# opencb/hpg-variant

Hardware: AMD Instinct MI355X
Metric: variants/s chi2 assoc (higher is better)
Workload: dtype u8

## Files before the change

### hpg-variant_amd/csrc/hpgv_capi.hip

```cpp
#include "hpgv_internal.h"
#include <cstdlib>

extern "C" {

const char *hpgv_version(void) { return "hpgv-mi355x 0.1 (gfx950)"; }

int hpgv_device_count(void) {
    int n = 0;
    if (hipGetDeviceCount(&n) != hipSuccess) return -1;
    return n;
}

const char *hpgv_last_error(const hpgv_ctx *ctx) { return ctx ? ctx->err.c_str() : g_create_error.c_str(); }

static void read_environment(hpgv_ctx *ctx) {
    auto num = [](const char *name, long lo, long hi, long *out) { const char *e = getenv(name); if (e && *e) { long v = atol(e); *out = v < lo ? lo : v > hi ? hi : v; } };
    num("HPGV_BATCH_COPY", 0, 1, &ctx->batch_copy);
    num("HPGV_BATCH_FUSED", 0, 1, &ctx->batch_fused);
    num("HPGV_STATS_ALL2", 0, 1, &ctx->stats_all2);
    num("HPGV_ASSOC_ROWS", 0, 1, &ctx->assoc_rows);
    num("HPGV_PINNED_NONCOHERENT", 0, 1, &ctx->pinned_noncoherent);
    num("HPGV_VMM_TRACE", 0, 1, &ctx->vmm_trace);
    num("HPGV_DECODE_TILES", 0, 1, &ctx->decode_tiles);
#ifdef HPGV_ABLATION
// ... 198 lines not shown
    } else if (!strcmp(key, "inflate_wave")) {
        if (value < 0 || value > 4) return fail(ctx, HPGV_ERR_INVALID, "inflate_wave must be 0 (lane per block), 1 (by the number of blocks), 2 (wave per block), 4 (wave per block, several symbols per round) or 3 (lane per block, symbol tables in LDS)");
        HPGV_SHIPPED_ONLY(value == 1 || value == 4, "inflate_wave other than 1 / 4 (a wave per block, several symbols per round)")
        ctx->inflate_wave = value;
    } else if (!strcmp(key, "tokenizer_tiles")) {
        if (value < 0 || value > 2) return fail(ctx, HPGV_ERR_INVALID, "tokenizer_tiles must be 2 (one sweep), 1 (two sweeps) or 0 (line by line)");
        HPGV_SHIPPED_ONLY(value == 1, "tokenizer_tiles other than 1 (two sweeps)")
        ctx->tokenizer_tiles = value;
    } else if (!strcmp(key, "fisher_width")) {
        if (value != 64 && value != 32 && value != 16 && value != 8) return fail(ctx, HPGV_ERR_INVALID, "fisher_width must be 64, 32, 16 or 8");
        HPGV_SHIPPED_ONLY(value == 16, "fisher_width other than 16")
        ctx->fisher_width = value;
    } else if (!strcmp(key, "batch_fused")) {
        ctx->batch_fused = value ? 1 : 0;
    } else if (!strcmp(key, "pipe_waves")) {
        if (value != 4 && value != 6 && value != 8) return fail(ctx, HPGV_ERR_INVALID, "pipe_waves must be 4, 6 or 8");
        HPGV_SHIPPED_ONLY(value == 4, "pipe_waves other than 4")
        ctx->pipe_waves = value;
    } else if (!strcmp(key, "persistent")) {
        HPGV_SHIPPED_ONLY(value == 0, "persistent = 1")
        ctx->persistent = value ? 1 : 0;
    } else if (!strcmp(key, "part_aligned_loads")) {
        HPGV_SHIPPED_ONLY(value == 0, "part_aligned_loads = 1")
        ctx->part_aligned = value ? 1 : 0;
    } else if (!strcmp(key, "blocks_per_cu")) {
        if (value < 1 || value > 8) return fail(ctx, HPGV_ERR_INVALID, "blocks_per_cu must be in 1..8");
        ctx->blocks_per_cu = value;
    } else {
        return fail(ctx, HPGV_ERR_INVALID, "unknown option '%s'", key);
    }
    return HPGV_OK;
}

// ... 480 lines not shown
```

### hpg-variant_amd/csrc/hpgv_internal.h

```cpp
#pragma once
#include "../../include/hpgv.h"
#include "hpgv_kernels.h"
#include "hpgv_tdt_stats_kernels.h"
#include "hpgv_epi_kernels.h"

#include <hip/hip_runtime.h>
#include <cctype>

#include <algorithm>
#include <atomic>
#include <cmath>
#include <cstdarg>
#include <cstdio>
#include <cstring>
#include <mutex>
#include <new>
#include <string>
#include <vector>

namespace { thread_local std::string g_create_error; }

struct DevBuf {
    void *p = nullptr;
    size_t cap = 0;
// ... 132 lines not shown
    long row_pad = 0;
    long vpw = 2;
    long nontemporal = 1;
    long profile = 0;
    std::mutex alias_mu;
    std::vector<std::pair<const char *, const char *>> text_alias;
    struct TextTiles { const char *d_text, *d_base; const void *d_tiles; uint64_t n_tiles; };
    std::vector<TextTiles> text_tiles;
    struct TextHeld { const char *host_text; Slot *slot; const char *d_text; const unsigned long long *d_line_off; int n_lines; };
    std::vector<TextHeld> text_held;
    long part_aligned = 0;
    long scan_unroll = 4;
    long persistent = 0;
    long blocks_per_cu = 8;
    long pipeline = 1;
    long pipe_waves = 4;
    long fisher_cut_exp = 22;
    long epi_complete = 1;
    long epi_pairs_mfma = 1;
    long epi_triples_mfma = 1;
    long epi_wide = 0;
    long epi_triples_1pass = 1;
    long scan_lds = 0;
    long fisher_width = 16;
    long inflate_wave = 1;
    long tokenizer_tiles = 1;
    long batch_copy = 0;
    long batch_fused = 1;
    long batch_lds_max = 65536;
    long stats_all2 = 1;
    long assoc_rows = 1;
// ... 239 lines not shown
```

### hpg-variant_amd/csrc/hpgv_kernels.h

```cpp
#pragma once
#include <hip/hip_runtime.h>
#include <stdint.h>

namespace hpgv {

__device__ __forceinline__ uint32_t nib_nonzero(uint32_t x) {
    uint32_t y = x | (x << 1);
    y = y | (y << 2);
    return y & 0x88888888u;
}
__device__ __forceinline__ uint32_t nib_not_f(uint32_t x) { return nib_nonzero(~x); }

__device__ __forceinline__ int wave_sum(int v) {
    v += __builtin_amdgcn_update_dpp(0, v, 0xB1, 0xF, 0xF, true);
    v += __builtin_amdgcn_update_dpp(0, v, 0x4E, 0xF, 0xF, true);
    v += __builtin_amdgcn_update_dpp(0, v, 0x141, 0xF, 0xF, true);
    v += __builtin_amdgcn_update_dpp(0, v, 0x140, 0xF, 0xF, true);
    return __builtin_amdgcn_readlane(v, 0) + __builtin_amdgcn_readlane(v, 16) +
           __builtin_amdgcn_readlane(v, 32) + __builtin_amdgcn_readlane(v, 48);
}

template <bool NT>
__device__ __forceinline__ uint4 load16(const uint4 *p);
template <bool NT>
__device__ __forceinline__ uint4 load16o(const uint8_t *__restrict__ base, uint32_t byte_off) {
    return load16<NT>(reinterpret_cast<const uint4 *>(base + byte_off));
}
template <bool NT>
__device__ __forceinline__ uint4 load16(const uint4 *p) {
    if constexpr (NT) {
        typedef uint32_t u32x4 __attribute__((ext_vector_type(4)));
        u32x4 t = __builtin_nontemporal_load(reinterpret_cast<const u32x4 *>(p));
        return make_uint4(t.x, t.y, t.z, t.w);
    } else {
// ... 48 lines not shown
        const int xxA = bA - (TA / 2 - validA), xxU = bU - (TU / 2 - validU);
        out.x = (TA - nzA) - validA + xxA;
        out.y = xxA;
        out.z = (TU - nzU) - validU + xxU;
        out.w = xxU;
    }
    if (lane == 0) *dst = out;
}

template <bool NT, int U, bool STRIDED>
__global__ __launch_bounds__(256) void k_assoc_scan(const uint8_t *__restrict__ gt, size_t pitch,
                                                    int n_variants, int chunksA, int chunks,
                                                    const uint8_t *__restrict__ is_x,
                                                    int4 *__restrict__ counts, int vpw) {
    const int lane = threadIdx.x & 63;
    const long wave = (long)blockIdx.x * (blockDim.x >> 6) + (threadIdx.x >> 6);
    const int slots = ((chunks + 64 * U - 1) / (64 * U)) * (64 * U);
    const int TA = 32 * chunksA;
    const int TU = 32 * (slots - chunksA);
    long v, v_end, v_step;
    if constexpr (STRIDED) { v = wave; v_end = n_variants; v_step = (long)gridDim.x * (blockDim.x >> 6); }
    else { v = wave * vpw; v_end = v + vpw < n_variants ? v + vpw : n_variants; v_step = 1; }

    for (; v < v_end; v += v_step) {
        const uint8_t *row = gt + (size_t)v * pitch;
        const bool x_row = (is_x != nullptr) && (__builtin_amdgcn_readfirstlane((int)is_x[v]) != 0);
        uint32_t pnz = 0, pnnf = 0, pbnz = 0;
        if (x_row) assoc_row<NT, U, true>(row, lane, chunksA, chunks, pnz, pnnf, pbnz);
        else       assoc_row<NT, U, false>(row, lane, chunksA, chunks, pnz, pnnf, pbnz);
        assoc_row_finish(x_row, lane, TA, TU, pnz, pnnf, pbnz, counts + v);
    }
}

struct AssocAcc { uint32_t pnz, pnnf, pbnz; };

template <int U, bool X>
__device__ __forceinline__ AssocAcc assoc_count_tile(const uint4 (&q)[U], int base, int lane, int chunksA,
                                                     AssocAcc a) {
#pragma unroll
    for (int u = 0; u < U; ++u) {
        const int c = base + u * 64 + lane;
        const uint32_t sh = (c < chunksA) ? 0u : 16u;
        const uint32_t w[4] = {q[u].x, q[u].y, q[u].z, q[u].w};
        uint32_t nz = 0, nnf = 0, bnz = 0;
#pragma unroll
        for (int k = 0; k < 4; ++k) {
            const uint32_t ind = nib_nonzero(w[k]);
            nz += __builtin_popcount(ind);
            nnf += __builtin_popcount(nib_not_f(w[k]));
            if constexpr (X) bnz += __builtin_popcount(ind & (ind >> 4) & 0x08080808u);
        }
        a.pnz += nz << sh;
        a.pnnf += nnf << sh;
        if constexpr (X) a.pbnz += bnz << sh;
    }
    return a;
}

template <bool NT, int U>
__device__ __forceinline__ void assoc_issue_tile(uint4 (&q)[U], const uint8_t *__restrict__ g0, size_t pitch,
                                                 int t, int ipr, int chunks, int lane) {
    const int r = t / ipr, base = (t - r * ipr) * 64 * U;
    const uint8_t *row = g0 + (size_t)r * pitch;
#pragma unroll
    for (int u = 0; u < U; ++u) {
        const int c = base + u * 64 + lane;
        q[u] = make_uint4(~0u, ~0u, ~0u, ~0u);
        if (c < chunks) q[u] = load16o<NT>(row, (uint32_t)c * 16u);
    }
}

template <int U>
__device__ __forceinline__ AssocAcc assoc_consume_tile(const uint4 (&q)[U], AssocAcc a, int t, int ipr, long v_begin,
                                                       int lane, int chunksA, int TA, int TU,
                                                       const uint8_t *__restrict__ is_x, int4 *__restrict__ counts) {
    const int r = t / ipr, it = t - r * ipr;
    const long v = v_begin + r;
    const bool x_row = (is_x != nullptr) && (__builtin_amdgcn_readfirstlane((int)is_x[v]) != 0);
    if (x_row) a = assoc_count_tile<U, true>(q, it * 64 * U, lane, chunksA, a);
    else       a = assoc_count_tile<U, false>(q, it * 64 * U, lane, chunksA, a);
    if (it == ipr - 1) {
        assoc_row_finish(x_row, lane, TA, TU, a.pnz, a.pnnf, a.pbnz, counts + v);
        a.pnz = a.pnnf = a.pbnz = 0;
    }
    return a;
}

template <bool NT, int U, int WAVES>
__global__ __launch_bounds__(256, WAVES) void k_assoc_scan_pipe(const uint8_t *__restrict__ gt, size_t pitch,
                                                         int n_variants, int chunksA, int chunks,
                                                         const uint8_t *__restrict__ is_x,
                                                         int4 *__restrict__ counts, int vpw) {
    const int lane = threadIdx.x & 63;
    const long wave = (long)blockIdx.x * (blockDim.x >> 6) + (threadIdx.x >> 6);
    const long v_begin = wave * vpw;
    if (v_begin >= n_variants) return;
    const int rows = (int)((v_begin + vpw <= n_variants) ? vpw : (n_variants - v_begin));
    const int ipr = (chunks + 64 * U - 1) / (64 * U);
    const int slots = ipr * 64 * U;
    const int TA = 32 * chunksA, TU = 32 * (slots - chunksA);
    const int n_tiles = rows * ipr;
    const uint8_t *g0 = gt + (size_t)v_begin * pitch;
    AssocAcc acc = {0u, 0u, 0u};
    uint4 qa[U], qb[U];
    assoc_issue_tile<NT, U>(qa, g0, pitch, 0, ipr, chunks, lane);
    for (int t = 0; t < n_tiles; t += 2) {
        if (t + 1 < n_tiles) assoc_issue_tile<NT, U>(qb, g0, pitch, t + 1, ipr, chunks, lane);
        acc = assoc_consume_tile<U>(qa, acc, t, ipr, v_begin, lane, chunksA, TA, TU, is_x, counts);
        if (t + 1 < n_tiles) {
            if (t + 2 < n_tiles) assoc_issue_tile<NT, U>(qa, g0, pitch, t + 2, ipr, chunks, lane);
            acc = assoc_consume_tile<U>(qb, acc, t + 1, ipr, v_begin, lane, chunksA, TA, TU, is_x, counts);
        }
    }
}

__device__ __forceinline__ double chisq_p_value(double x) {
    if (x != x) return x;
    if (x <= 0.0) return 1.0;
    const double y = x / 2.0;
    double P;
    if (y > 0.5) P = 1.0 - erfc(sqrt(y));
    else         P = erf(sqrt(y));
    return 1.0 - P;
}

__device__ __forceinline__ double assoc_odds(int A1, int A2, int U1, int U2) {
// ... 431 lines not shown
```

### hpg-variant_amd/csrc/hpgv_scan_capi.hip

```cpp
#include "hpgv_internal.h"
#include <type_traits>
#include "hpgv_inherit_kernels.h"

namespace {

unsigned scan_blocks(const hpgv_ctx *ctx, int n_variants) {
    const long waves = ((long)n_variants + ctx->vpw - 1) / ctx->vpw;
    return (unsigned)((waves + 3) / 4);
}

const char *const kAligned16 = "device buffers must be 16-byte aligned";
int scan_checks(hpgv_ctx *ctx, int n_variants, const void *d_gt, const void *d_out, uintptr_t out_mask, const char *align_text, bool *go) {
    *go = false;
    if (n_variants < 0 || (n_variants > 0 && (!d_gt || !d_out))) return fail(ctx, HPGV_ERR_INVALID, "bad scan arguments");
    if (n_variants == 0) return HPGV_OK;
    if (((uintptr_t)d_gt & 15) || ((uintptr_t)d_out & out_mask)) return fail(ctx, HPGV_ERR_INVALID, "%s", align_text);
    *go = true;
    return HPGV_OK;
}

template <typename F>
void launch_nt(const hpgv_ctx *ctx, F &&f) {
    if (ctx->nontemporal) f(std::true_type{}); else f(std::false_type{});
}

}

extern "C" {


static Layout *pick_layout(hpgv_ctx *ctx, int which) {
    switch (which) {
        case HPGV_LAYOUT_ASSOC: return &ctx->assoc;
        case HPGV_LAYOUT_TDT: return &ctx->tdt;
        case HPGV_LAYOUT_STATS: return &ctx->stats;
        case HPGV_LAYOUT_STATS_GROUPS: return &ctx->sgroups;
        case HPGV_LAYOUT_MENDEL: return &ctx->mendel;
        case HPGV_LAYOUT_EPI: return &ctx->assoc;
        default: return nullptr;
// ... 99 lines not shown
                        int32_t *d_counts, void *stream) {
    ctx = first_member(ctx);
    if (!ctx) return HPGV_ERR_INVALID;
    if (!ctx->assoc.set) return fail(ctx, HPGV_ERR_STATE, "hpgv_set_cohort has not been called");
    bool go;
    if (const int rc = scan_checks(ctx, n_variants, d_gt, d_counts, 15, kAligned16, &go); rc || !go) return rc;
    DeviceGuard g(ctx->device);
    const Layout &L = ctx->assoc;
    const int vpw = (int)ctx->vpw;
    unsigned blocks = scan_blocks(ctx, n_variants);
    if (ctx->persistent) {
        const unsigned cap = (unsigned)(ctx->n_cus * ctx->blocks_per_cu);
        const unsigned need = (unsigned)(((long)n_variants + 3) / 4);
        blocks = need < cap ? need : cap;
    }
    hipStream_t st = (hipStream_t)stream;
    const uint8_t *gt = d_gt;
    int4 *out = (int4 *)d_counts;
    const int cA = ctx->chunksA, ch = L.chunks;
    const size_t pitch = L.pitch;
#define HPGV_LAUNCH_PIPE(NT, U, W)                                                                \
    hipLaunchKernelGGL((hpgv::k_assoc_scan_pipe<NT, U, W>), dim3(blocks), dim3(256), 0, st, gt, pitch, \
                       n_variants, cA, ch, d_is_x, out, vpw)
#ifndef HPGV_ABLATION
    return launch_profiled(ctx, st, 0, [&] { HPGV_LAUNCH_PIPE(true, 4, 4); });
#else
#define HPGV_LAUNCH_ASSOC(NT, U, S)                                                              \
    hipLaunchKernelGGL((hpgv::k_assoc_scan<NT, U, S>), dim3(blocks), dim3(256), 0, st, gt, pitch, \
                       n_variants, cA, ch, d_is_x, out, vpw)
#define HPGV_DISPATCH_U(NT, S)                                                                   \
    switch (ctx->scan_unroll) {                                                                  \
        case 4: HPGV_LAUNCH_ASSOC(NT, 4, S); break;                                              \
        case 10: HPGV_LAUNCH_ASSOC(NT, 10, S); break;                                            \
        case 12: HPGV_LAUNCH_ASSOC(NT, 12, S); break;                                            \
        case 16: HPGV_LAUNCH_ASSOC(NT, 16, S); break;                                            \
        default: HPGV_LAUNCH_ASSOC(NT, 8, S); break;                                             \
    }
#define HPGV_PIPE_W(NT, U)                                                                       \
    do {                                                                                         \
        if (ctx->pipe_waves == 8) { HPGV_LAUNCH_PIPE(NT, U, 8); }                                \
        else if (ctx->pipe_waves == 6) { HPGV_LAUNCH_PIPE(NT, U, 6); }                           \
        else { HPGV_LAUNCH_PIPE(NT, U, 4); }                                                     \
    } while (0)
    if (ctx->pipeline && !ctx->persistent)
        return launch_profiled(ctx, st, 0, [&] {
            if (ctx->nontemporal) {
                if (ctx->scan_unroll <= 4) HPGV_PIPE_W(true, 4); else HPGV_PIPE_W(true, 5);
            } else {
                if (ctx->scan_unroll <= 4) HPGV_PIPE_W(false, 4); else HPGV_PIPE_W(false, 5);
            }
        });
    return launch_profiled(ctx, st, 0, [&] {
        if (ctx->nontemporal) {
            if (ctx->persistent) { HPGV_DISPATCH_U(true, true) } else { HPGV_DISPATCH_U(true, false) }
        } else {
            if (ctx->persistent) { HPGV_DISPATCH_U(false, true) } else { HPGV_DISPATCH_U(false, false) }
        }
    });
#undef HPGV_DISPATCH_U
#undef HPGV_PIPE_W
#undef HPGV_LAUNCH_ASSOC
#endif
#undef HPGV_LAUNCH_PIPE
}

int hpgv_assoc_chisq_dev(hpgv_ctx *ctx, const int32_t *d_counts, int n_variants, double *d_odds,
                         double *d_chisq, double *d_p, void *stream) {
    ctx = first_member(ctx);
    if (!ctx) return HPGV_ERR_INVALID;
    if (n_variants < 0 || (n_variants > 0 && (!d_counts || !d_odds || !d_chisq || !d_p)))
        return fail(ctx, HPGV_ERR_INVALID, "bad chisq arguments");
    if (n_variants == 0) return HPGV_OK;
    DeviceGuard g(ctx->device);
    hipStream_t st = (hipStream_t)stream;
    return launch_profiled(ctx, st, 1, [&] {
        hipLaunchKernelGGL(hpgv::k_assoc_chisq, dim3((n_variants + 255) / 256), dim3(256), 0, st,
                           (const int4 *)d_counts, n_variants, d_odds, d_chisq, d_p);
// ... 57 lines not shown
    hipStream_t st = (hipStream_t)stream;
    return launch_profiled(ctx, st, 1, [&] {
        hipLaunchKernelGGL(hpgv::k_tdt_stats, dim3((n_variants + 255) / 256), dim3(256), 0, st,
                           (const int2 *)d_tu, n_variants, d_odds, d_chisq, d_p);
    });
}


static int stats_scan(hpgv_ctx *ctx, const Layout &L, const uint8_t *d_gt, int n_variants, uint32_t off, int chunks, size_t lds,
                      int32_t *d_counts8, hipStream_t st) {
    bool go;
    if (const int rc = scan_checks(ctx, n_variants, d_gt, d_counts8, 15, kAligned16, &go); rc || !go) return rc;
    DeviceGuard g(ctx->device);
    const int vpw = (int)ctx->vpw;
    const unsigned blocks = scan_blocks(ctx, n_variants);
    return launch_profiled(ctx, st, 0, [&] {
        launch_nt(ctx, [&](auto NT) {
            constexpr bool nt = decltype(NT)::value;
            if (ctx->pipeline)
                hipLaunchKernelGGL((hpgv::k_stats_scan_hs<nt>), dim3(blocks), dim3(256), nt ? lds : 0, st, d_gt, L.pitch, n_variants, off, chunks, (int4 *)d_counts8, vpw);
            else
                hipLaunchKernelGGL((hpgv::k_stats_scan<nt, kScanUnroll>), dim3(blocks), dim3(256), 0, st, d_gt, L.pitch, n_variants, off, chunks, (int4 *)d_counts8, vpw);
        });
    });
}

int hpgv_stats_scan_dev(hpgv_ctx *ctx, const uint8_t *d_gt, int n_variants, int32_t *d_counts8, void *stream) {
    ctx = first_member(ctx);
    if (!ctx) return HPGV_ERR_INVALID;
    if (!ctx->stats.set) return fail(ctx, HPGV_ERR_STATE, "hpgv_set_stats_cohort has not been called");
    const Layout &L = ctx->stats;
    const size_t scan_lds = ctx->scan_lds > 0 ? (size_t)ctx->scan_lds : (L.pitch >= 6656 ? (size_t)49152 : (size_t)0);
    return stats_scan(ctx, L, d_gt, n_variants, 0u, L.chunks, scan_lds, d_counts8, (hipStream_t)stream);
}

int hpgv_stats_scan_group_dev(hpgv_ctx *ctx, const uint8_t *d_gt, int n_variants, int group, int32_t *d_counts8, void *stream) {
    ctx = first_member(ctx);
    if (!ctx) return HPGV_ERR_INVALID;
    if (!ctx->sgroups.set) return fail(ctx, HPGV_ERR_STATE, "hpgv_set_stats_groups has not been called");
    if (group < 0 || (size_t)group >= ctx->sg_off.size()) return fail(ctx, HPGV_ERR_INVALID, "group %d out of range", group);
    const int chunks = (int)(round_up((size_t)ctx->sg_size[(size_t)group], 16) / 16);
    return stats_scan(ctx, ctx->sgroups, d_gt, n_variants, ctx->sg_off[(size_t)group], chunks, 0, d_counts8, (hipStream_t)stream);
}

int hpgv_stats_hwe_dev(hpgv_ctx *ctx, const int32_t *d_counts8, int n_variants, double *d_chi2,
                       double *d_p, void *stream) {
    ctx = first_member(ctx);
// ... 161 lines not shown
```

### hpg-variant_amd/csrc/hpgv_tdt_stats_kernels.h

```cpp
#pragma once
#include "hpgv_kernels.h"

#include <algorithm>
#include <cstring>
#include <string>
#include <vector>

namespace hpgv {

__host__ __device__ __forceinline__ int mendel_code(bool is_x_male, int f1, int f2, int m1, int m2, int c1, int c2) {
    const bool f_ref = !f1 && !f2, f_alt = f1 && f2, m_ref = !m1 && !m2, m_alt = m1 && m2;
    const bool c_ref = !c1 && !c2, c_alt = c1 && c2;
    if (is_x_male) return (c_alt && m_ref) ? 9 : (c_ref && m_alt) ? 10 : 0;
    if (!c_ref && !c_alt) return (f_ref && m_ref) ? 1 : (f_alt && m_alt) ? 2 : 0;
    if (c_ref) return (f_alt && m_alt) ? 5 : m_alt ? 3 : f_alt ? 4 : 0;
    return (f_ref && m_ref) ? 8 : f_ref ? 6 : m_ref ? 7 : 0;
}

__host__ __device__ __forceinline__ bool tdt_parents_usable(int f1, int f2, int m1, int m2) {
    if (f1 == 0xF || f2 == 0xF || m1 == 0xF || m2 == 0xF) return false;
    if (f1 == f2 && m1 == m2) return false;
    if ((f1 && !f2) || (m1 && !m2)) return false;
    return true;
}
// ... 84 lines not shown
}

__device__ __forceinline__ uint32_t popcount_bytes(uint32_t w) {
    w = w - ((w >> 1) & 0x55555555u);
    w = (w & 0x33333333u) + ((w >> 2) & 0x33333333u);
    return (w + (w >> 4)) & 0x0F0F0F0Fu;
}

template <bool X>
__device__ __forceinline__ uint32_t tdt4_diff(const TdtLuts &L, uint32_t f, uint32_t m, uint32_t c, uint32_t male) {
    uint32_t w1, w2;
    tdt4_words<X>(L, f, m, c, male, w1, w2);
    return ((popcount_bytes(w1) | 0x80808080u) - popcount_bytes(w2)) ^ 0x80808080u;
}

template <bool NT, int U>
__global__ __launch_bounds__(256) void k_tdt_scan(const uint8_t *__restrict__ gt, size_t pitch, int n_variants,
                                                  int pchunks , TdtLuts luts,
                                                  const uint8_t *__restrict__ male_plane,
                                                  int n_slow, const int32_t *__restrict__ slow_off,
                                                  const uint8_t *__restrict__ slow_male, int slow_base,
                                                  const uint8_t *__restrict__ is_x, int2 *__restrict__ tu, int vpw) {
    const int lane = threadIdx.x & 63;
    const long wave = (long)blockIdx.x * (blockDim.x >> 6) + (threadIdx.x >> 6);
    const long v_begin = wave * vpw;
    for (int i = 0; i < vpw; ++i) {
        const long v = v_begin + i;
        if (v >= n_variants) break;
        const uint8_t *rowb = gt + (size_t)v * pitch;
        const uint32_t plane = (uint32_t)pchunks * 16u;
        const bool x_row = (is_x != nullptr) && (__builtin_amdgcn_readfirstlane((int)is_x[v]) != 0);
        int t1 = 0, t2 = 0;
        for (int base = 0; base < pchunks; base += 64 * U) {
            uint4 qf[U], qm[U], qc[U];
#pragma unroll
            for (int u = 0; u < U; ++u) {
                const int c = base + u * 64 + lane;
                qf[u] = make_uint4(0x80808080u, 0x80808080u, 0x80808080u, 0x80808080u);
                qm[u] = make_uint4(0x20202020u, 0x20202020u, 0x20202020u, 0x20202020u);
                qc[u] = make_uint4(0x04040404u, 0x04040404u, 0x04040404u, 0x04040404u);
                if (c < pchunks) {
                    qf[u] = load16o<NT>(rowb, (uint32_t)c * 16u);
                    qm[u] = load16o<NT>(rowb, (uint32_t)c * 16u + plane);
                    qc[u] = load16o<NT>(rowb, (uint32_t)c * 16u + 2u * plane);
                }
            }
// ... 109 lines not shown
                    if (tdt_parents_usable(P[f][0], P[f][1], P[m][0], P[m][1]))
                        st = tdt_child(P[f][0], P[f][1], P[m][0], P[m][1], C[c][0], C[c][1], x == 1, st);
                    w1[x][f][m][c] = st.t1; w2[x][f][m][c] = st.t2;
                }
    uint8_t pair[16], c1[8], c2[8];
    if (!encode(w1[0], w2[0], true, true, pair, c1, c2)) return false;
    pack(pair, c1, c2, out.autosome);
    if (!encode(w1[1], w2[1], true, false, pair, c1, c2)) return false;
    pack(pair, c1, c2, out.xmale_t1);
    if (!encode(w1[1], w2[1], false, true, pair, c1, c2)) return false;
    pack(pair, c1, c2, out.xmale_t2);
    return true;
}

}

struct TdtPlan {
    int n_fast = 0, n_slow_families = 0;
    int pchunks = 0;
    int p16 = 0;
    int slow_base = 0;
    int max_children = 0;
    std::vector<int32_t> fast_family, slow_family;
    TdtLuts luts{};
    uint8_t *d_male_plane = nullptr;
    int32_t *d_slow_off = nullptr;
    uint8_t *d_slow_male = nullptr;

    void release() {
        if (d_male_plane) (void)hipFree(d_male_plane);
// ... 63 lines not shown
            !up((void **)&d_slow_off, slow_off.data(), slow_off.size() * sizeof(int32_t)) ||
            !up((void **)&d_slow_male, slow_male.data(), slow_male.size())) {
            why = "hipMalloc/hipMemcpy of the TDT plan failed";
            release();
            return 3;
        }
        return 0;
    }

    void launch_scan(const uint8_t *d_gt, size_t pitch, int n_variants, const uint8_t *d_is_x, int2 *d_tu,
                     int vpw, bool nt, hipStream_t st) const {
        const long waves = ((long)n_variants + vpw - 1) / vpw;
        const unsigned blocks = (unsigned)((waves + 3) / 4);
        constexpr int U = 4;
        if (nt)
            hipLaunchKernelGGL((k_tdt_scan<true, U>), dim3(blocks), dim3(256), 0, st, d_gt, pitch, n_variants, pchunks, luts,
                               d_male_plane, n_slow_families, d_slow_off, d_slow_male, slow_base, d_is_x, d_tu, vpw);
        else
            hipLaunchKernelGGL((k_tdt_scan<false, U>), dim3(blocks), dim3(256), 0, st, d_gt, pitch, n_variants, pchunks, luts,
                               d_male_plane, n_slow_families, d_slow_off, d_slow_male, slow_base, d_is_x, d_tu, vpw);
    }
};

template <bool NT, int U>
__global__ __launch_bounds__(256) void k_stats_scan(const uint8_t *__restrict__ gt, size_t pitch, int n_variants,
                                                    uint32_t row_off ,
                                                    int chunks, int4 *__restrict__ out8, int vpw) {
    const int lane = threadIdx.x & 63;
    const long wave = (long)blockIdx.x * (blockDim.x >> 6) + (threadIdx.x >> 6);
    const long v_begin = wave * vpw;
    for (int i = 0; i < vpw; ++i) {
        const long v = v_begin + i;
        if (v >= n_variants) break;
        const uint8_t *row = gt + (size_t)v * pitch + row_off;
        int cnt[8] = {0, 0, 0, 0, 0, 0, 0, 0};
        for (int base = 0; base < chunks; base += 64 * U) {
            uint4 q[U];
#pragma unroll
            for (int u = 0; u < U; ++u) {
                const int c = base + u * 64 + lane;
                q[u] = make_uint4(0u, 0u, 0u, 0u);
                if (c < chunks) q[u] = load16o<NT>(row, (uint32_t)c * 16u);
            }
#pragma unroll
            for (int u = 0; u < U; ++u) {
// ... 25 lines not shown
__device__ __forceinline__ void stats_count_tile(const uint4 (&q)[4], StatsAcc &a) {
    const uint32_t w[16] = {q[0].x, q[0].y, q[0].z, q[0].w, q[1].x, q[1].y, q[1].z, q[1].w,
                            q[2].x, q[2].y, q[2].z, q[2].w, q[3].x, q[3].y, q[3].z, q[3].w};
    uint32_t t2a, t2b, t4a, t4b, t8a, t8b, s16;
    csa(t2a, a.ones, a.ones, w[0], w[1]);   csa(t2b, a.ones, a.ones, w[2], w[3]);   csa(t4a, a.twos, a.twos, t2a, t2b);
    csa(t2a, a.ones, a.ones, w[4], w[5]);   csa(t2b, a.ones, a.ones, w[6], w[7]);   csa(t4b, a.twos, a.twos, t2a, t2b);
    csa(t8a, a.fours, a.fours, t4a, t4b);
    csa(t2a, a.ones, a.ones, w[8], w[9]);   csa(t2b, a.ones, a.ones, w[10], w[11]); csa(t4a, a.twos, a.twos, t2a, t2b);
    csa(t2a, a.ones, a.ones, w[12], w[13]); csa(t2b, a.ones, a.ones, w[14], w[15]); csa(t4b, a.twos, a.twos, t2a, t2b);
    csa(t8b, a.fours, a.fours, t4a, t4b);
    csa(s16, a.eights, a.eights, t8a, t8b);
#pragma unroll
    for (int b = 0; b < 8; ++b) a.c16[b] += __builtin_popcount(s16 & (0x01010101u << b));
}

template <bool NT>
__device__ __forceinline__ void stats_issue_tile(uint4 (&q)[4], const uint8_t *__restrict__ g0, size_t pitch, int t, int ipr,
                                                 int chunks, int lane) {
    const int r = t / ipr, base = (t - r * ipr) * 256;
    const uint8_t *row = g0 + (size_t)r * pitch;
#pragma unroll
    for (int u = 0; u < 4; ++u) {
        const int c = base + u * 64 + lane;
        q[u] = make_uint4(0u, 0u, 0u, 0u);
        if (c < chunks) q[u] = load16o<NT>(row, (uint32_t)c * 16u);
    }
}

__device__ __forceinline__ void stats_consume_tile(const uint4 (&q)[4], StatsAcc &a, int t, int ipr, long v_begin, int lane,
                                                   int4 *__restrict__ out8) {
    stats_count_tile(q, a);
    const int r = t / ipr;
    if (t - r * ipr == ipr - 1) {
        int s[8], c[8];
#pragma unroll
        for (int b = 0; b < 8; ++b) {
            const uint32_t m = 0x01010101u << b;
            c[b] = 16 * a.c16[b] + 8 * __builtin_popcount(a.eights & m) + 4 * __builtin_popcount(a.fours & m) +
                   2 * __builtin_popcount(a.twos & m) + __builtin_popcount(a.ones & m);
            a.c16[b] = 0;
        }
        if (ipr * 4096 < 65536) {
#pragma unroll
            for (int b = 0; b < 8; b += 2) {
                const int two = wave_sum(c[b] | (c[b + 1] << 16));
                s[b] = two & 0xFFFF; s[b + 1] = (int)((uint32_t)two >> 16);
            }
        } else {
#pragma unroll
            for (int b = 0; b < 8; ++b) s[b] = wave_sum(c[b]);
        }
        a.ones = a.twos = a.fours = a.eights = 0u;
        const long v = v_begin + r;
        if (lane == 0) {
            out8[2 * v] = make_int4(s[0], s[1], s[2], s[3]);
            out8[2 * v + 1] = make_int4(s[4], s[4] + s[5], 2 * s[0] + s[1] + s[2] + s[6], 2 * s[3] + s[1] + s[2] + s[7]);
        }
    }
}

template <bool NT>
__global__ __launch_bounds__(256) void k_stats_scan_hs(const uint8_t *__restrict__ gt, size_t pitch, int n_variants,
                                                       uint32_t row_off, int chunks, int4 *__restrict__ out8, int vpw) {
    const int lane = threadIdx.x & 63;
    const long wave = (long)blockIdx.x * (blockDim.x >> 6) + (threadIdx.x >> 6);
    const long v_begin = wave * vpw;
    if (v_begin >= n_variants) return;
    const int rows = (int)((v_begin + vpw <= n_variants) ? vpw : (n_variants - v_begin));
    const int ipr = chunks > 0 ? (chunks + 255) / 256 : 1;
    const int n_tiles = rows * ipr;
    const uint8_t *g0 = gt + (size_t)v_begin * pitch + row_off;
    StatsAcc acc;
    acc.ones = acc.twos = acc.fours = acc.eights = 0u;
#pragma unroll
    for (int b = 0; b < 8; ++b) acc.c16[b] = 0;
    uint4 qa[4], qb[4];
    stats_issue_tile<NT>(qa, g0, pitch, 0, ipr, chunks, lane);
    for (int t = 0; t < n_tiles; t += 2) {
        if (t + 1 < n_tiles) stats_issue_tile<NT>(qb, g0, pitch, t + 1, ipr, chunks, lane);
        stats_consume_tile(qa, acc, t, ipr, v_begin, lane, out8);
        if (t + 1 < n_tiles) {
            if (t + 2 < n_tiles) stats_issue_tile<NT>(qa, g0, pitch, t + 2, ipr, chunks, lane);
            stats_consume_tile(qb, acc, t + 1, ipr, v_begin, lane, out8);
        }
    }
}

constexpr int SAMPLE_STATS_ROWS = 128;
static __global__ __launch_bounds__(256) void k_sample_missing(const uint8_t *__restrict__ gt, size_t pitch, int n_variants,
                                                        int chunks, int n_samples, int32_t *__restrict__ missing) {
    const int lane = threadIdx.x & 63;
    const int tile = blockIdx.x * (blockDim.x >> 6) + (threadIdx.x >> 6);
    const int c = tile * 64 + lane;
    const long v0 = (long)blockIdx.y * SAMPLE_STATS_ROWS;
    if (tile * 64 >= chunks) return;
    uint32_t acc[4] = {0, 0, 0, 0};
    const int rows = (int)((v0 + SAMPLE_STATS_ROWS <= n_variants) ? SAMPLE_STATS_ROWS : (n_variants - v0));
    if (c < chunks) {
// ... 47 lines not shown
__device__ __forceinline__ uint32_t mendel4(const MendelLuts &L, uint32_t f, uint32_t m, uint32_t c, uint32_t male) {
    const uint32_t idx = (m << 2) | f;
    uint32_t z = mendel_err4(L.autosome, idx, c);
    if constexpr (X) {
        const uint32_t zx = mendel_err4(L.xmale, idx, c);
        z = (male & zx) | (~male & z);
    }
    return any3(z);
}

template <bool NT, int U>
__global__ __launch_bounds__(256) void k_mendel_scan(const uint8_t *__restrict__ gt, size_t pitch, int n_variants,
                                                     int pchunks, MendelLuts luts, const uint8_t *__restrict__ male_plane,
                                                     const uint8_t *__restrict__ is_x, int32_t *__restrict__ errors, int vpw) {
    const int lane = threadIdx.x & 63;
    const long wave = (long)blockIdx.x * (blockDim.x >> 6) + (threadIdx.x >> 6);
    const long v_begin = wave * vpw;
    const uint32_t plane = (uint32_t)pchunks * 16u;
    for (int i = 0; i < vpw; ++i) {
        const long v = v_begin + i;
        if (v >= n_variants) break;
        const uint8_t *rowb = gt + (size_t)v * pitch;
        const bool x_row = (is_x != nullptr) && (__builtin_amdgcn_readfirstlane((int)is_x[v]) != 0);
        int n = 0;
        for (int base = 0; base < pchunks; base += 64 * U) {
            uint4 qf[U], qm[U], qc[U];
#pragma unroll
            for (int u = 0; u < U; ++u) {
                const int c = base + u * 64 + lane;
                qf[u] = qm[u] = qc[u] = make_uint4(0x03030303u, 0x03030303u, 0x03030303u, 0x03030303u);
                if (c < pchunks) {
                    qf[u] = load16o<NT>(rowb, (uint32_t)c * 16u);
                    qm[u] = load16o<NT>(rowb, (uint32_t)c * 16u + plane);
                    qc[u] = load16o<NT>(rowb, (uint32_t)c * 16u + 2u * plane);
                }
            }
#pragma unroll
            for (int u = 0; u < U; ++u) {
// ... 113 lines not shown
```

Measured before the change: 137.4 million.

## Add multi-set tile pipelining with row-size-dependent waves-per-EU forms for scans

Rewrites the assoc and stats pipelined scan kernels to rotate through two to four register tile sets, so loads for later tiles are issued while earlier tiles are counted. Each kernel gets an explicit waves-per-EU occupancy target chosen from the row byte width. Tail tiles are masked instead of branch-guarded per load, which allows unconditional loads from a clamped address. The per-row X-chromosome flag is now read with a scalar constant-address load, and the wave index is made uniform. The risks are higher register pressure from more tile sets and a more complex tile-walk state.

```diff
diff --git a/hpg-variant_amd/csrc/hpgv_capi.hip b/hpg-variant_amd/csrc/hpgv_capi.hip
--- a/hpg-variant_amd/csrc/hpgv_capi.hip
+++ b/hpg-variant_amd/csrc/hpgv_capi.hip
@@ -236,9 +236,13 @@
     } else if (!strcmp(key, "batch_fused")) {
         ctx->batch_fused = value ? 1 : 0;
     } else if (!strcmp(key, "pipe_waves")) {
-        if (value != 4 && value != 6 && value != 8) return fail(ctx, HPGV_ERR_INVALID, "pipe_waves must be 4, 6 or 8");
-        HPGV_SHIPPED_ONLY(value == 4, "pipe_waves other than 4")
+        if (value != 0 && (value < 2 || value > 8 || value == 7)) return fail(ctx, HPGV_ERR_INVALID, "pipe_waves must be 0 (the shipped form of each scan), 2 .. 6 or 8");
+        HPGV_SHIPPED_ONLY(value == 0, "pipe_waves other than 0")
         ctx->pipe_waves = value;
+    } else if (!strcmp(key, "pipe_sets")) {
+        if (value != 0 && (value < 2 || value > 4)) return fail(ctx, HPGV_ERR_INVALID, "pipe_sets must be 0 (the shipped form of each scan), 2, 3 or 4");
+        HPGV_SHIPPED_ONLY(value == 0, "pipe_sets other than 0")
+        ctx->pipe_sets = value;
     } else if (!strcmp(key, "persistent")) {
         HPGV_SHIPPED_ONLY(value == 0, "persistent = 1")
         ctx->persistent = value ? 1 : 0;
diff --git a/hpg-variant_amd/csrc/hpgv_internal.h b/hpg-variant_amd/csrc/hpgv_internal.h
--- a/hpg-variant_amd/csrc/hpgv_internal.h
+++ b/hpg-variant_amd/csrc/hpgv_internal.h
@@ -170,7 +170,8 @@
     long persistent = 0;
     long blocks_per_cu = 8;
     long pipeline = 1;
-    long pipe_waves = 4;
+    long pipe_waves = 0;
+    long pipe_sets = 0;
     long fisher_cut_exp = 22;
     long epi_complete = 1;
     long epi_pairs_mfma = 1;
diff --git a/hpg-variant_amd/csrc/hpgv_kernels.h b/hpg-variant_amd/csrc/hpgv_kernels.h
--- a/hpg-variant_amd/csrc/hpgv_kernels.h
+++ b/hpg-variant_amd/csrc/hpgv_kernels.h
@@ -1,6 +1,7 @@
 #pragma once
 #include <hip/hip_runtime.h>
 #include <stdint.h>
+#include "hpgv_scan_walk.h"
 
 namespace hpgv {
 
@@ -18,6 +19,17 @@
     v += __builtin_amdgcn_update_dpp(0, v, 0x140, 0xF, 0xF, true);
     return __builtin_amdgcn_readlane(v, 0) + __builtin_amdgcn_readlane(v, 16) +
            __builtin_amdgcn_readlane(v, 32) + __builtin_amdgcn_readlane(v, 48);
+}
+
+__device__ __forceinline__ long scan_wave_index() {
+    return (long)blockIdx.x * (blockDim.x >> 6) + __builtin_amdgcn_readfirstlane((int)(threadIdx.x >> 6));
+}
+
+__device__ __forceinline__ uint32_t scalar_byte(const uint8_t *__restrict__ p, long i) {
+    const uintptr_t a = (uintptr_t)(p + i);
+    typedef const __attribute__((address_space(4))) uint32_t *const_u32_ptr;
+    const uint32_t w = *(const_u32_ptr)(a & ~(uintptr_t)3);
+    return (w >> (8u * (uint32_t)(a & 3))) & 0xFFu;
 }
 
 template <bool NT>
@@ -96,7 +108,7 @@
                                                     const uint8_t *__restrict__ is_x,
                                                     int4 *__restrict__ counts, int vpw) {
     const int lane = threadIdx.x & 63;
-    const long wave = (long)blockIdx.x * (blockDim.x >> 6) + (threadIdx.x >> 6);
+    const long wave = scan_wave_index();
     const int slots = ((chunks + 64 * U - 1) / (64 * U)) * (64 * U);
     const int TA = 32 * chunksA;
     const int TU = 32 * (slots - chunksA);
@@ -106,7 +118,7 @@
 
     for (; v < v_end; v += v_step) {
         const uint8_t *row = gt + (size_t)v * pitch;
-        const bool x_row = (is_x != nullptr) && (__builtin_amdgcn_readfirstlane((int)is_x[v]) != 0);
+        const bool x_row = (is_x != nullptr) && (scalar_byte(is_x, v) != 0u);
         uint32_t pnz = 0, pnnf = 0, pbnz = 0;
         if (x_row) assoc_row<NT, U, true>(row, lane, chunksA, chunks, pnz, pnnf, pbnz);
         else       assoc_row<NT, U, false>(row, lane, chunksA, chunks, pnz, pnnf, pbnz);
@@ -116,17 +128,17 @@
 
 struct AssocAcc { uint32_t pnz, pnnf, pbnz; };
 
-template <int U, bool X>
-__device__ __forceinline__ AssocAcc assoc_count_tile(const uint4 (&q)[U], int base, int lane, int chunksA,
-                                                     AssocAcc a) {
+template <int U, bool X, bool LAST>
+__device__ __forceinline__ AssocAcc assoc_count_tile(const uint4 (&q)[U], int leftA, int left, int lane, AssocAcc a) {
 #pragma unroll
     for (int u = 0; u < U; ++u) {
-        const int c = base + u * 64 + lane;
-        const uint32_t sh = (c < chunksA) ? 0u : 16u;
-        const uint32_t w[4] = {q[u].x, q[u].y, q[u].z, q[u].w};
+        const int c = u * 64 + lane;
+        const uint32_t sh = (c < leftA) ? 0u : 16u;
+        uint32_t w[4] = {q[u].x, q[u].y, q[u].z, q[u].w};
         uint32_t nz = 0, nnf = 0, bnz = 0;
 #pragma unroll
         for (int k = 0; k < 4; ++k) {
+            if constexpr (LAST) w[k] = (c < left) ? w[k] : ~0u;
             const uint32_t ind = nib_nonzero(w[k]);
             nz += __builtin_popcount(ind);
             nnf += __builtin_popcount(nib_not_f(w[k]));
@@ -137,6 +149,11 @@
         if constexpr (X) a.pbnz += bnz << sh;
     }
     return a;
+}
+
+template <int U, bool X>
+__device__ __forceinline__ AssocAcc assoc_count_tile(const uint4 (&q)[U], int base, int lane, int chunksA, AssocAcc a) {
+    return assoc_count_tile<U, X, false>(q, chunksA - base, 0, lane, a);
 }
 
 template <bool NT, int U>
@@ -152,46 +169,77 @@
     }
 }
 
+struct ScanIssue {
+    const uint8_t *row;
+    const uint8_t *idle;
+    size_t pitch;
+    ScanWalk w;
+    int left;
+    int chunks, ipr;
+};
+
+template <bool NT, int U>
+__device__ __forceinline__ void scan_issue_tile(uint4 (&q)[U], ScanIssue &s, int lane) {
+    const bool live = s.left > 0;
+    const int base = s.w.tile * 64 * U;
+    const uint8_t *p = live ? s.row + (uint32_t)base * 16u : s.idle;
+    const uint32_t limit = live ? scan_walk_limit(s.chunks, base) : 0u;
+#pragma unroll
+    for (int u = 0; u < U; ++u) q[u] = load16o<NT>(p, scan_walk_lane_off(lane, u, limit));
+    --s.left;
+    if (scan_walk_step(&s.w, s.ipr)) s.row += s.pitch;
+}
+
 template <int U>
-__device__ __forceinline__ AssocAcc assoc_consume_tile(const uint4 (&q)[U], AssocAcc a, int t, int ipr, long v_begin,
-                                                       int lane, int chunksA, int TA, int TU,
+__device__ __forceinline__ AssocAcc assoc_consume_tile(const uint4 (&q)[U], AssocAcc a, ScanWalk &w, int ipr, long v_begin,
+                                                       int lane, int chunksA, int chunks, int TA, int TU,
                                                        const uint8_t *__restrict__ is_x, int4 *__restrict__ counts) {
-    const int r = t / ipr, it = t - r * ipr;
-    const long v = v_begin + r;
-    const bool x_row = (is_x != nullptr) && (__builtin_amdgcn_readfirstlane((int)is_x[v]) != 0);
-    if (x_row) a = assoc_count_tile<U, true>(q, it * 64 * U, lane, chunksA, a);
-    else       a = assoc_count_tile<U, false>(q, it * 64 * U, lane, chunksA, a);
-    if (it == ipr - 1) {
+    const long v = v_begin + w.row;
+    const int base = w.tile * 64 * U;
+    const bool x_row = (is_x != nullptr) && (scalar_byte(is_x, v) != 0u);
+    if (w.tile == ipr - 1) {
+        if (x_row) a = assoc_count_tile<U, true, true>(q, chunksA - base, chunks - base, lane, a);
+        else       a = assoc_count_tile<U, false, true>(q, chunksA - base, chunks - base, lane, a);
         assoc_row_finish(x_row, lane, TA, TU, a.pnz, a.pnnf, a.pbnz, counts + v);
         a.pnz = a.pnnf = a.pbnz = 0;
-    }
+    } else {
+        if (x_row) a = assoc_count_tile<U, true, false>(q, chunksA - base, chunks - base, lane, a);
+        else       a = assoc_count_tile<U, false, false>(q, chunksA - base, chunks - base, lane, a);
+    }
+    scan_walk_step(&w, ipr);
     return a;
 }
 
-template <bool NT, int U, int WAVES>
-__global__ __launch_bounds__(256, WAVES) void k_assoc_scan_pipe(const uint8_t *__restrict__ gt, size_t pitch,
-                                                         int n_variants, int chunksA, int chunks,
-                                                         const uint8_t *__restrict__ is_x,
-                                                         int4 *__restrict__ counts, int vpw) {
+template <bool NT, int U, int W, int SETS>
+__global__ __launch_bounds__(256) __attribute__((amdgpu_waves_per_eu(W, W)))
+void k_assoc_scan_pipe(const uint8_t *__restrict__ gt, size_t pitch, int n_variants, int chunksA, int chunks,
+                       const uint8_t *__restrict__ is_x, int4 *__restrict__ counts, int vpw) {
+    static_assert(SETS >= 2 && SETS <= 4, "two to four tile sets");
     const int lane = threadIdx.x & 63;
-    const long wave = (long)blockIdx.x * (blockDim.x >> 6) + (threadIdx.x >> 6);
-    const long v_begin = wave * vpw;
-    if (v_begin >= n_variants) return;
+    const long v_begin = scan_wave_index() * vpw;
+    if (v_begin >= n_variants || chunks <= 0) return;
     const int rows = (int)((v_begin + vpw <= n_variants) ? vpw : (n_variants - v_begin));
-    const int ipr = (chunks + 64 * U - 1) / (64 * U);
+    const int ipr = scan_walk_ipr(chunks, 64 * U);
     const int slots = ipr * 64 * U;
     const int TA = 32 * chunksA, TU = 32 * (slots - chunksA);
     const int n_tiles = rows * ipr;
-    const uint8_t *g0 = gt + (size_t)v_begin * pitch;
+    ScanIssue is;
+    is.row = is.idle = gt + (size_t)v_begin * pitch;
+    is.pitch = pitch; is.w = ScanWalk{0, 0}; is.left = n_tiles; is.chunks = chunks; is.ipr = ipr;
+    ScanWalk cw = {0, 0};
     AssocAcc acc = {0u, 0u, 0u};
-    uint4 qa[U], qb[U];
-    assoc_issue_tile<NT, U>(qa, g0, pitch, 0, ipr, chunks, lane);
-    for (int t = 0; t < n_tiles; t += 2) {
-        if (t + 1 < n_tiles) assoc_issue_tile<NT, U>(qb, g0, pitch, t + 1, ipr, chunks, lane);
-        acc = assoc_consume_tile<U>(qa, acc, t, ipr, v_begin, lane, chunksA, TA, TU, is_x, counts);
-        if (t + 1 < n_tiles) {
-            if (t + 2 < n_tiles) assoc_issue_tile<NT, U>(qa, g0, pitch, t + 2, ipr, chunks, lane);
-            acc = assoc_consume_tile<U>(qb, acc, t + 1, ipr, v_begin, lane, chunksA, TA, TU, is_x, counts);
+    uint4 q[SETS][U];
+#pragma unroll
+    for (int s = 0; s < SETS - 1; ++s) {
+        scan_issue_tile<NT, U>(q[s], is, lane);
+        __builtin_amdgcn_sched_barrier(0);
+    }
+    for (int t = 0; t < n_tiles; t += SETS) {
+#pragma unroll
+        for (int s = 0; s < SETS; ++s) {
+            scan_issue_tile<NT, U>(q[(s + SETS - 1) % SETS], is, lane);
+            if (t + s < n_tiles)
+                acc = assoc_consume_tile<U>(q[s], acc, cw, ipr, v_begin, lane, chunksA, chunks, TA, TU, is_x, counts);
         }
     }
 }
diff --git a/hpg-variant_amd/csrc/hpgv_scan_capi.hip b/hpg-variant_amd/csrc/hpgv_scan_capi.hip
--- a/hpg-variant_amd/csrc/hpgv_scan_capi.hip
+++ b/hpg-variant_amd/csrc/hpgv_scan_capi.hip
@@ -23,6 +23,20 @@
 void launch_nt(const hpgv_ctx *ctx, F &&f) {
     if (ctx->nontemporal) f(std::true_type{}); else f(std::false_type{});
 }
+
+int assoc_scan_form(size_t row_bytes) { return row_bytes < 8192 ? 82 : row_bytes < 24576 ? 32 : 23; }
+int stats_scan_form(size_t row_bytes) { return row_bytes < 6656 ? 82 : row_bytes < 24576 ? 34 : 23; }
+bool assoc_form_built(int f) { return f == 23 || f == 24 || f == 32 || f == 33 || f == 34 || f == 42 || f == 43 || f == 52 || f == 53 || f == 62 || f == 63 || f == 82; }
+bool stats_form_built(int f) { return f == 23 || f == 24 || f == 32 || f == 33 || f == 34 || f == 42 || f == 43 || f == 52 || f == 53 || f == 62 || f == 82; }
+#ifdef HPGV_ABLATION
+int scan_form(const hpgv_ctx *ctx, int shipped) {
+    return (int)((ctx->pipe_waves ? ctx->pipe_waves : shipped / 10) * 10 + (ctx->pipe_sets ? ctx->pipe_sets : shipped % 10));
+}
+#define HPGV_OTHER_FORM(...) __VA_ARGS__
+#else
+int scan_form(const hpgv_ctx *, int shipped) { return shipped; }
+#define HPGV_OTHER_FORM(...)
+#endif
 
 }
 
@@ -152,16 +166,33 @@
         const unsigned need = (unsigned)(((long)n_variants + 3) / 4);
         blocks = need < cap ? need : cap;
     }
+    if (!assoc_form_built(scan_form(ctx, assoc_scan_form(L.pitch))))
+        return fail(ctx, HPGV_ERR_UNSUPPORTED, "the assoc scan has no form of %ld waves per SIMD x %ld tile sets", ctx->pipe_waves, ctx->pipe_sets);
     hipStream_t st = (hipStream_t)stream;
     const uint8_t *gt = d_gt;
     int4 *out = (int4 *)d_counts;
     const int cA = ctx->chunksA, ch = L.chunks;
     const size_t pitch = L.pitch;
-#define HPGV_LAUNCH_PIPE(NT, U, W)                                                                \
-    hipLaunchKernelGGL((hpgv::k_assoc_scan_pipe<NT, U, W>), dim3(blocks), dim3(256), 0, st, gt, pitch, \
+#define HPGV_LAUNCH_PIPE(NT, U, W, S)                                                             \
+    hipLaunchKernelGGL((hpgv::k_assoc_scan_pipe<NT, U, W, S>), dim3(blocks), dim3(256), 0, st, gt, pitch, \
                        n_variants, cA, ch, d_is_x, out, vpw)
+#define HPGV_PIPE_FORMS()                                                                         \
+    switch (scan_form(ctx, assoc_scan_form(pitch))) {                                             \
+        case 82: HPGV_LAUNCH_PIPE(true, 4, 8, 2); break;                                          \
+        case 32: HPGV_LAUNCH_PIPE(true, 4, 3, 2); break;                                          \
+        HPGV_OTHER_FORM(case 24: HPGV_LAUNCH_PIPE(true, 4, 2, 4); break;                          \
+                        case 33: HPGV_LAUNCH_PIPE(true, 4, 3, 3); break;                          \
+                        case 34: HPGV_LAUNCH_PIPE(true, 4, 3, 4); break;                          \
+                        case 42: HPGV_LAUNCH_PIPE(true, 4, 4, 2); break;                          \
+                        case 43: HPGV_LAUNCH_PIPE(true, 4, 4, 3); break;                          \
+                        case 52: HPGV_LAUNCH_PIPE(true, 4, 5, 2); break;                          \
+                        case 53: HPGV_LAUNCH_PIPE(true, 4, 5, 3); break;                          \
+                        case 62: HPGV_LAUNCH_PIPE(true, 4, 6, 2); break;                          \
+                        case 63: HPGV_LAUNCH_PIPE(true, 4, 6, 3); break;)                         \
+        default: HPGV_LAUNCH_PIPE(true, 4, 2, 3); break;                                          \
+    }
 #ifndef HPGV_ABLATION
-    return launch_profiled(ctx, st, 0, [&] { HPGV_LAUNCH_PIPE(true, 4, 4); });
+    return launch_profiled(ctx, st, 0, [&] { HPGV_PIPE_FORMS(); });
 #else
 #define HPGV_LAUNCH_ASSOC(NT, U, S)                                                              \
     hipLaunchKernelGGL((hpgv::k_assoc_scan<NT, U, S>), dim3(blocks), dim3(256), 0, st, gt, pitch, \
@@ -174,18 +205,14 @@
         case 16: HPGV_LAUNCH_ASSOC(NT, 16, S); break;                                            \
         default: HPGV_LAUNCH_ASSOC(NT, 8, S); break;                                             \
     }
-#define HPGV_PIPE_W(NT, U)                                                                       \
-    do {                                                                                         \
-        if (ctx->pipe_waves == 8) { HPGV_LAUNCH_PIPE(NT, U, 8); }                                \
-        else if (ctx->pipe_waves == 6) { HPGV_LAUNCH_PIPE(NT, U, 6); }                           \
-        else { HPGV_LAUNCH_PIPE(NT, U, 4); }                                                     \
-    } while (0)
     if (ctx->pipeline && !ctx->persistent)
         return launch_profiled(ctx, st, 0, [&] {
-            if (ctx->nontemporal) {
-                if (ctx->scan_unroll <= 4) HPGV_PIPE_W(true, 4); else HPGV_PIPE_W(true, 5);
+            if (!ctx->nontemporal) {
+                if (ctx->scan_unroll <= 4) HPGV_LAUNCH_PIPE(false, 4, 4, 2); else HPGV_LAUNCH_PIPE(false, 5, 4, 2);
+            } else if (ctx->scan_unroll > 4) {
+                HPGV_LAUNCH_PIPE(true, 5, 4, 2);
             } else {
-                if (ctx->scan_unroll <= 4) HPGV_PIPE_W(false, 4); else HPGV_PIPE_W(false, 5);
+                HPGV_PIPE_FORMS();
             }
         });
     return launch_profiled(ctx, st, 0, [&] {
@@ -196,9 +223,9 @@
         }
     });
 #undef HPGV_DISPATCH_U
-#undef HPGV_PIPE_W
 #undef HPGV_LAUNCH_ASSOC
 #endif
+#undef HPGV_PIPE_FORMS
 #undef HPGV_LAUNCH_PIPE
 }
 
@@ -286,13 +313,33 @@
     DeviceGuard g(ctx->device);
     const int vpw = (int)ctx->vpw;
     const unsigned blocks = scan_blocks(ctx, n_variants);
+    if (!stats_form_built(scan_form(ctx, stats_scan_form((size_t)chunks * 16))))
+        return fail(ctx, HPGV_ERR_UNSUPPORTED, "the stats scan has no form of %ld waves per SIMD x %ld tile sets", ctx->pipe_waves, ctx->pipe_sets);
     return launch_profiled(ctx, st, 0, [&] {
         launch_nt(ctx, [&](auto NT) {
             constexpr bool nt = decltype(NT)::value;
-            if (ctx->pipeline)
-                hipLaunchKernelGGL((hpgv::k_stats_scan_hs<nt>), dim3(blocks), dim3(256), nt ? lds : 0, st, d_gt, L.pitch, n_variants, off, chunks, (int4 *)d_counts8, vpw);
-            else
+#define HPGV_LAUNCH_HS(W, S)                                                                      \
+    hipLaunchKernelGGL((hpgv::k_stats_scan_hs<nt, W, S>), dim3(blocks), dim3(256), nt ? lds : 0, st, d_gt, L.pitch, n_variants, off, chunks, (int4 *)d_counts8, vpw)
+#ifdef HPGV_ABLATION
+            if (!ctx->pipeline) {
                 hipLaunchKernelGGL((hpgv::k_stats_scan<nt, kScanUnroll>), dim3(blocks), dim3(256), 0, st, d_gt, L.pitch, n_variants, off, chunks, (int4 *)d_counts8, vpw);
+                return;
+            }
+#endif
+            switch (scan_form(ctx, stats_scan_form((size_t)chunks * 16))) {
+                case 82: HPGV_LAUNCH_HS(8, 2); break;
+                case 34: HPGV_LAUNCH_HS(3, 4); break;
+                HPGV_OTHER_FORM(case 24: HPGV_LAUNCH_HS(2, 4); break;
+                                case 32: HPGV_LAUNCH_HS(3, 2); break;
+                                case 33: HPGV_LAUNCH_HS(3, 3); break;
+                                case 42: HPGV_LAUNCH_HS(4, 2); break;
+                                case 43: HPGV_LAUNCH_HS(4, 3); break;
+                                case 52: HPGV_LAUNCH_HS(5, 2); break;
+                                case 53: HPGV_LAUNCH_HS(5, 3); break;
+                                case 62: HPGV_LAUNCH_HS(6, 2); break;)
+                default: HPGV_LAUNCH_HS(2, 3); break;
+            }
+#undef HPGV_LAUNCH_HS
         });
     });
 }
@@ -302,7 +349,7 @@
     if (!ctx) return HPGV_ERR_INVALID;
     if (!ctx->stats.set) return fail(ctx, HPGV_ERR_STATE, "hpgv_set_stats_cohort has not been called");
     const Layout &L = ctx->stats;
-    const size_t scan_lds = ctx->scan_lds > 0 ? (size_t)ctx->scan_lds : (L.pitch >= 6656 ? (size_t)49152 : (size_t)0);
+    const size_t scan_lds = ctx->scan_lds > 0 ? (size_t)ctx->scan_lds : (size_t)0;
     return stats_scan(ctx, L, d_gt, n_variants, 0u, L.chunks, scan_lds, d_counts8, (hipStream_t)stream);
 }
 
diff --git a/hpg-variant_amd/csrc/hpgv_scan_walk.h b/hpg-variant_amd/csrc/hpgv_scan_walk.h
--- /dev/null
+++ b/hpg-variant_amd/csrc/hpgv_scan_walk.h
@@ -0,0 +1,28 @@
+#pragma once
+#include <stdint.h>
+
+#if defined(__HIPCC__) || defined(__CUDACC__)
+#define HPGV_HD __host__ __device__ __forceinline__
+#else
+#define HPGV_HD static inline
+#endif
+
+typedef struct ScanWalk {
+    int row;
+    int tile;
+} ScanWalk;
+
+HPGV_HD int scan_walk_ipr(int chunks, int tile_chunks) { return chunks > 0 ? (chunks + tile_chunks - 1) / tile_chunks : 1; }
+
+HPGV_HD int scan_walk_step(ScanWalk *w, int ipr) {
+    if (++w->tile < ipr) return 0;
+    w->tile = 0;
+    ++w->row;
+    return 1;
+}
+
+HPGV_HD uint32_t scan_walk_limit(int chunks, int base) { return (uint32_t)(chunks - 1 - base) * 16u; }
+HPGV_HD uint32_t scan_walk_lane_off(int lane, int u, uint32_t limit) {
+    const uint32_t o = (uint32_t)lane * 16u + (uint32_t)u * 1024u;
+    return o < limit ? o : limit;
+}
diff --git a/hpg-variant_amd/csrc/hpgv_tdt_stats_kernels.h b/hpg-variant_amd/csrc/hpgv_tdt_stats_kernels.h
--- a/hpg-variant_amd/csrc/hpgv_tdt_stats_kernels.h
+++ b/hpg-variant_amd/csrc/hpgv_tdt_stats_kernels.h
@@ -122,22 +122,22 @@
     return ((popcount_bytes(w1) | 0x80808080u) - popcount_bytes(w2)) ^ 0x80808080u;
 }
 
-template <bool NT, int U>
-__global__ __launch_bounds__(256) void k_tdt_scan(const uint8_t *__restrict__ gt, size_t pitch, int n_variants,
+template <bool NT, int U, int W>
+__global__ __launch_bounds__(256) __attribute__((amdgpu_waves_per_eu(W, W)))
+void k_tdt_scan(const uint8_t *__restrict__ gt, size_t pitch, int n_variants,
                                                   int pchunks , TdtLuts luts,
                                                   const uint8_t *__restrict__ male_plane,
                                                   int n_slow, const int32_t *__restrict__ slow_off,
                                                   const uint8_t *__restrict__ slow_male, int slow_base,
                                                   const uint8_t *__restrict__ is_x, int2 *__restrict__ tu, int vpw) {
     const int lane = threadIdx.x & 63;
-    const long wave = (long)blockIdx.x * (blockDim.x >> 6) + (threadIdx.x >> 6);
-    const long v_begin = wave * vpw;
+    const long v_begin = scan_wave_index() * vpw;
     for (int i = 0; i < vpw; ++i) {
         const long v = v_begin + i;
         if (v >= n_variants) break;
         const uint8_t *rowb = gt + (size_t)v * pitch;
         const uint32_t plane = (uint32_t)pchunks * 16u;
-        const bool x_row = (is_x != nullptr) && (__builtin_amdgcn_readfirstlane((int)is_x[v]) != 0);
+        const bool x_row = (is_x != nullptr) && (scalar_byte(is_x, v) != 0u);
         int t1 = 0, t2 = 0;
         for (int base = 0; base < pchunks; base += 64 * U) {
             uint4 qf[U], qm[U], qc[U];
@@ -277,6 +277,8 @@
 }
 
 }
+
+constexpr int kTdtWaves = 4;
 
 struct TdtPlan {
     int n_fast = 0, n_slow_families = 0;
@@ -370,10 +372,10 @@
         const unsigned blocks = (unsigned)((waves + 3) / 4);
         constexpr int U = 4;
         if (nt)
-            hipLaunchKernelGGL((k_tdt_scan<true, U>), dim3(blocks), dim3(256), 0, st, d_gt, pitch, n_variants, pchunks, luts,
+            hipLaunchKernelGGL((k_tdt_scan<true, U, kTdtWaves>), dim3(blocks), dim3(256), 0, st, d_gt, pitch, n_variants, pchunks, luts,
                                d_male_plane, n_slow_families, d_slow_off, d_slow_male, slow_base, d_is_x, d_tu, vpw);
         else
-            hipLaunchKernelGGL((k_tdt_scan<false, U>), dim3(blocks), dim3(256), 0, st, d_gt, pitch, n_variants, pchunks, luts,
+            hipLaunchKernelGGL((k_tdt_scan<false, U, kTdtWaves>), dim3(blocks), dim3(256), 0, st, d_gt, pitch, n_variants, pchunks, luts,
                                d_male_plane, n_slow_families, d_slow_off, d_slow_male, slow_base, d_is_x, d_tu, vpw);
     }
 };
@@ -383,8 +385,7 @@
                                                     uint32_t row_off ,
                                                     int chunks, int4 *__restrict__ out8, int vpw) {
     const int lane = threadIdx.x & 63;
-    const long wave = (long)blockIdx.x * (blockDim.x >> 6) + (threadIdx.x >> 6);
-    const long v_begin = wave * vpw;
+    const long v_begin = scan_wave_index() * vpw;
     for (int i = 0; i < vpw; ++i) {
         const long v = v_begin + i;
         if (v >= n_variants) break;
@@ -440,24 +441,20 @@
     for (int b = 0; b < 8; ++b) a.c16[b] += __builtin_popcount(s16 & (0x01010101u << b));
 }
 
-template <bool NT>
-__device__ __forceinline__ void stats_issue_tile(uint4 (&q)[4], const uint8_t *__restrict__ g0, size_t pitch, int t, int ipr,
-                                                 int chunks, int lane) {
-    const int r = t / ipr, base = (t - r * ipr) * 256;
-    const uint8_t *row = g0 + (size_t)r * pitch;
-#pragma unroll
-    for (int u = 0; u < 4; ++u) {
-        const int c = base + u * 64 + lane;
-        q[u] = make_uint4(0u, 0u, 0u, 0u);
-        if (c < chunks) q[u] = load16o<NT>(row, (uint32_t)c * 16u);
-    }
-}
-
-__device__ __forceinline__ void stats_consume_tile(const uint4 (&q)[4], StatsAcc &a, int t, int ipr, long v_begin, int lane,
-                                                   int4 *__restrict__ out8) {
-    stats_count_tile(q, a);
-    const int r = t / ipr;
-    if (t - r * ipr == ipr - 1) {
+template <bool LAST>
+__device__ __forceinline__ void stats_mask_tile(uint4 (&q)[4], int left, int lane) {
+    if constexpr (LAST) {
+#pragma unroll
+        for (int u = 0; u < 4; ++u)
+            if (u * 64 + lane >= left) q[u] = make_uint4(0u, 0u, 0u, 0u);
+    }
+}
+
+__device__ __forceinline__ void stats_consume_tile(uint4 (&q)[4], StatsAcc &a, ScanWalk &w, int ipr, int chunks, long v_begin,
+                                                   int lane, int4 *__restrict__ out8) {
+    if (w.tile == ipr - 1) {
+        stats_mask_tile<true>(q, chunks - w.tile * 256, lane);
+        stats_count_tile(q, a);
         int s[8], c[8];
 #pragma unroll
         for (int b = 0; b < 8; ++b) {
@@ -477,37 +474,48 @@
             for (int b = 0; b < 8; ++b) s[b] = wave_sum(c[b]);
         }
         a.ones = a.twos = a.fours = a.eights = 0u;
-        const long v = v_begin + r;
+        const long v = v_begin + w.row;
         if (lane == 0) {
             out8[2 * v] = make_int4(s[0], s[1], s[2], s[3]);
             out8[2 * v + 1] = make_int4(s[4], s[4] + s[5], 2 * s[0] + s[1] + s[2] + s[6], 2 * s[3] + s[1] + s[2] + s[7]);
         }
-    }
-}
-
-template <bool NT>
-__global__ __launch_bounds__(256) void k_stats_scan_hs(const uint8_t *__restrict__ gt, size_t pitch, int n_variants,
-                                                       uint32_t row_off, int chunks, int4 *__restrict__ out8, int vpw) {
+    } else {
+        stats_count_tile(q, a);
+    }
+    scan_walk_step(&w, ipr);
+}
+
+template <bool NT, int W, int SETS>
+__global__ __launch_bounds__(256) __attribute__((amdgpu_waves_per_eu(W, W)))
+void k_stats_scan_hs(const uint8_t *__restrict__ gt, size_t pitch, int n_variants, uint32_t row_off, int chunks,
+                     int4 *__restrict__ out8, int vpw) {
+    static_assert(SETS >= 2 && SETS <= 4, "two to four tile sets");
     const int lane = threadIdx.x & 63;
-    const long wave = (long)blockIdx.x * (blockDim.x >> 6) + (threadIdx.x >> 6);
-    const long v_begin = wave * vpw;
+    const long v_begin = scan_wave_index() * vpw;
     if (v_begin >= n_variants) return;
     const int rows = (int)((v_begin + vpw <= n_variants) ? vpw : (n_variants - v_begin));
-    const int ipr = chunks > 0 ? (chunks + 255) / 256 : 1;
+    const int ipr = scan_walk_ipr(chunks, 256);
     const int n_tiles = rows * ipr;
-    const uint8_t *g0 = gt + (size_t)v_begin * pitch + row_off;
+    ScanIssue is;
+    is.idle = gt + (size_t)v_begin * pitch;
+    is.row = is.idle + row_off;
+    is.pitch = pitch; is.w = ScanWalk{0, 0}; is.left = chunks > 0 ? n_tiles : 0; is.chunks = chunks; is.ipr = ipr;
+    ScanWalk cw = {0, 0};
     StatsAcc acc;
     acc.ones = acc.twos = acc.fours = acc.eights = 0u;
 #pragma unroll
     for (int b = 0; b < 8; ++b) acc.c16[b] = 0;
-    uint4 qa[4], qb[4];
-    stats_issue_tile<NT>(qa, g0, pitch, 0, ipr, chunks, lane);
-    for (int t = 0; t < n_tiles; t += 2) {
-        if (t + 1 < n_tiles) stats_issue_tile<NT>(qb, g0, pitch, t + 1, ipr, chunks, lane);
-        stats_consume_tile(qa, acc, t, ipr, v_begin, lane, out8);
-        if (t + 1 < n_tiles) {
-            if (t + 2 < n_tiles) stats_issue_tile<NT>(qa, g0, pitch, t + 2, ipr, chunks, lane);
-            stats_consume_tile(qb, acc, t + 1, ipr, v_begin, lane, out8);
+    uint4 q[SETS][4];
+#pragma unroll
+    for (int s = 0; s < SETS - 1; ++s) {
+        scan_issue_tile<NT, 4>(q[s], is, lane);
+        __builtin_amdgcn_sched_barrier(0);
+    }
+    for (int t = 0; t < n_tiles; t += SETS) {
+#pragma unroll
+        for (int s = 0; s < SETS; ++s) {
+            scan_issue_tile<NT, 4>(q[(s + SETS - 1) % SETS], is, lane);
+            if (t + s < n_tiles) stats_consume_tile(q[s], acc, cw, ipr, chunks, v_begin, lane, out8);
         }
     }
 }
@@ -585,14 +593,13 @@
                                                      int pchunks, MendelLuts luts, const uint8_t *__restrict__ male_plane,
                                                      const uint8_t *__restrict__ is_x, int32_t *__restrict__ errors, int vpw) {
     const int lane = threadIdx.x & 63;
-    const long wave = (long)blockIdx.x * (blockDim.x >> 6) + (threadIdx.x >> 6);
-    const long v_begin = wave * vpw;
+    const long v_begin = scan_wave_index() * vpw;
     const uint32_t plane = (uint32_t)pchunks * 16u;
     for (int i = 0; i < vpw; ++i) {
         const long v = v_begin + i;
         if (v >= n_variants) break;
         const uint8_t *rowb = gt + (size_t)v * pitch;
-        const bool x_row = (is_x != nullptr) && (__builtin_amdgcn_readfirstlane((int)is_x[v]) != 0);
+        const bool x_row = (is_x != nullptr) && (scalar_byte(is_x, v) != 0u);
         int n = 0;
         for (int base = 0; base < pchunks; base += 64 * U) {
             uint4 qf[U], qm[U], qc[U];
```

Measured after the change: 139.0 million, median of 6. No clear change (+1.2%).
